# stevengiacalone/triceratops

Hardware: AMD Instinct MI355X
Metric: light-curve-point x sample evals/sec (higher is better)
Workload: dtype f64

## Files before the change

### triceratops_amd/csrc/trx_cells.hpp

```cpp
#pragma once
#include <hip/hip_runtime.h>
#include <math.h>

#include <cstddef>
#include <cstdint>

#include "../../include/trx.h"
#include "trx_device.hpp"
#include "trx_internal.hpp"

namespace {

using namespace trx;

constexpr int MODE_LNL = 0;
constexpr int MODE_GRID = 1;

struct RowsArgs {
    int model, flags;
    const double* time;
    const double* flux;
    int n_time;
    double sigma;
    const double* params;
// ... 373 lines not shown
                }
            }
            hdr[kHdrGrid + lane] = dpt;
            hdr[kHdrG + lane] = g;
        }
        if (lane == 0) {
            hdr[kHdrFlat] = acc;
            hdr[kHdrHmin] = INFINITY;
            hdr[kHdrXmax] = -INFINITY;
            hdr[kHdrProbe] = 1.0;
        }
    }
    {
        const int l = lane, nt = a.n_time;
        bool ok = a.use_stencil && nt >= 64 && a.S >= 2 && a.exptime > 0.0;
        double dt = 0.0, t0 = 0.0;
        if (ok) {
            t0 = a.time[0];
            dt = (a.time[nt - 1] - t0) / (double)(nt - 1);
            double dev = 0.0, big = 0.0;
            for (int j = l; j < nt; j += 64) {
                const double t = a.time[j];
                dev = fmax(dev, fabs(t - fma((double)j, dt, t0)));
                big = fmax(big, fabs(t));
            }
#pragma unroll
            for (int o = 32; o > 0; o >>= 1) {
                dev = fmax(dev, __shfl_xor(dev, o, 64));
                big = fmax(big, __shfl_xor(big, o, 64));
            }
            ok = dt > 0.0 && dev <= 4.0 * 2.220446049250313e-16 * fmax(big, dt);
        }
        const double u = ok ? dt / a.exptime : 1.0;
        ok = ok && u <= 0.3 && 0.5 / u <= 0.5 * kStM + 0.5;
        double w = 0.0, pmax = 0.0;
        if (ok && l <= 2 * kStM + 1) {
            const int i = l - kStM;
            for (int sidx = 1; sidx <= a.S; ++sidx) {
                const double x = (((double)sidx - 0.5) * a.rS - 0.5) / u;
                double num = 1.0, den = 1.0;
                for (int k = -kStM; k <= kStM; ++k) {
                    if (l == 2 * kStM + 1) num *= fabs(x - (double)k);
                    else if (k != i) { num *= x - (double)k; den *= (double)(i - k); }
                }
                if (l == 2 * kStM + 1) pmax = fmax(pmax, num);
                else w += num / den;
            }
            w *= a.rS;
        }
        pmax = __shfl(pmax, 2 * kStM + 1, 64);
        double wabs = (l <= 2 * kStM) ? fabs(w) : 0.0;
#pragma unroll
        for (int o = 32; o > 0; o >>= 1) wabs += __shfl_xor(wabs, o, 64);
        ok = ok && wabs <= 3.0;
        if (l <= 2 * kStM) hdr[kHdrStW + l] = ok ? w : 0.0;
        if (l == 0) {
            double radius = 0.0;
            if (ok) {
                radius = 1.1 * 2.0 * u * ((double)kStM + pow(pmax * 1e15, 1.0 / (2.0 * kStM + 1.0)));
                if (!(radius > 0.0 && radius <= 40.0)) radius = 0.0;
            }
            hdr[kHdrStRadius] = radius;
            if (a.memo) *a.memo = (radius > 0.0) ? 2 : 1;
        }
    }
}

constexpr unsigned long long kUnwrittenBits = 0x7ff8dead0badc0deull;

template <bool SEC>
__device__ __forceinline__ void rowc_body(const RowsArgs& a)
{
    __shared__ RowC rows_out[64];
    const int lane = threadIdx.x;
    const long n = a.n_dev ? *a.n_dev : a.n;
    const long nblk = (n + 63) / 64;
    if (blockIdx.x == gridDim.x - 1) {
        launch_header(a, n);
        return;
    }
    const bool quick = SEC && a.out_sec == nullptr;
    int* list = a.scan_list;
    unsigned long long* count = a.scan_count;
    for (long blk = blockIdx.x; blk < nblk; blk += gridDim.x - 1) {
        const long base = blk * 64;
        const int nb = (int)((n - base < 64) ? (n - base) : 64);
        bool open = false;
        if (lane < nb) {
            RowC c, sc;
            double ysec, fdil;
            row_constants(a, n, base + lane, c, quick, sc, ysec, fdil);
            if (quick) {
#ifndef TRX_SEC_FULL_SCAN
                const Limb L{sc.cle, sc.cld, sc.ced};
                const double ts = __dadd_rn(__dmul_rn(0.1 / 24.0, 12.0), -0.05);
                const double f = exposure_flux(sc, L, ts, 0.0, 1, 1.0, 1.0, false, a.tiers);
                const double m = (f + ysec) / (1.0 + ysec);
                const double depth = 1.0 - (m + fdil) / (1.0 + fdil);
                if (!(depth < 1.5 * a.sigma)) c.excl = 1.0;
                else open = true;
#else
                open = true;
#endif
            }
            const double* src = reinterpret_cast<const double*>(&c);
            double* stage = reinterpret_cast<double*>(&rows_out[lane]);
#pragma unroll
            for (int q = 0; q < kRowDoubles; ++q) stage[q] = src[q];
        }
        if (quick) {
            const unsigned long long mo = __ballot(open);
            if (mo) {
                unsigned long long at = 0;
                if (lane == 0) at = atomicAdd(count, (unsigned long long)__popcll(mo));
                at = __shfl(at, 0, 64);
                const unsigned long long slot = at + (unsigned long long)lanes_below(mo);
                if (open && slot <= (unsigned long long)a.n) list[slot] = (int)(base + lane);
            }
        }
        if (a.mark_unwritten && lane < nb) a.out[base + lane] = __longlong_as_double((long long)kUnwrittenBits);
        __syncthreads();
        {
            const double* src = reinterpret_cast<const double*>(rows_out);
            double* out = a.rowc + base * kRowDoubles;
            for (int i = lane; i < nb * kRowDoubles; i += 64) out[i] = src[i];
        }
        __syncthreads();
    }
}

template <bool SEC>
__global__ __launch_bounds__(64) void rowc_kernel(RowsArgs a)
{
    rowc_body<SEC>(a);
}

__global__ __launch_bounds__(64) void rowc_kernel_star(RowsArgs common, BranchTab bt)
{
    const RowsArgs a = star_args(common, bt, 0);
    if (a.need_sec) rowc_body<true>(a);
    else rowc_body<false>(a);
}

template <int E>
__device__ __forceinline__ void sec_scan_body(const RowsArgs& a)
{
    __shared__ RowC srows[E];
    __shared__ double secmin[E];
    __shared__ int secnan[E];
    const int lane = threadIdx.x;
    const long n = a.n_dev ? *a.n_dev : a.n;
    const bool all_rows = a.out_sec != nullptr;
    const int* list = a.scan_list;
    const long nu = all_rows ? n : (long)*a.scan_count;
    for (long e0 = (long)blockIdx.x * E; e0 < nu; e0 += (long)gridDim.x * E) {
        const int ne = (int)((nu - e0 < E) ? (nu - e0) : E);
        long row = 0;
        double ysec = 0.0, fdil = 0.0;
        if (lane < ne) {
            row = all_rows ? e0 + lane : (long)list[e0 + lane];
            row = (row >= 0 && row < n) ? row : 0;
            RowC unused;
            row_constants<false>(a, n, row, unused, true, srows[lane], ysec, fdil);
            secmin[lane] = INFINITY;
            secnan[lane] = 0;
        }
        __syncthreads();
        for (int it = lane; it < ne * kSecPoints; it += 64) {
            const int ri = it / kSecPoints, j = it - ri * kSecPoints;
            const RowC sc = srows[ri];
            const Limb L{sc.cle, sc.cld, sc.ced};
            double ts = __dadd_rn(__dmul_rn(0.1 / 24.0, (double)j), -0.05);
            if (j == kSecPoints - 1) ts = 0.05;
            const double f = exposure_flux(sc, L, ts, 0.0, 1, 1.0, 1.0, false, a.tiers);
            if (f != f) atomicOr(&secnan[ri], 1);
            else __hip_atomic_fetch_min(&secmin[ri], f, __ATOMIC_RELAXED, __HIP_MEMORY_SCOPE_WORKGROUP);
        }
        __syncthreads();
        if (lane < ne) {
            double m = secnan[lane] ? NAN : secmin[lane];
            m = (m + ysec) / (1.0 + ysec);
            const double secdepth = 1.0 - (m + fdil) / (1.0 + fdil);
            a.rowc[row * kRowDoubles + (kRowDoubles - 1)] = (secdepth < 1.5 * a.sigma) ? 0.0 : 1.0;
            if (a.out_sec) a.out_sec[row] = secdepth;
        }
        __syncthreads();
    }
}

template <int E>
__global__ __launch_bounds__(64) void sec_scan_kernel(RowsArgs a)
{
    sec_scan_body<E>(a);
}

struct BranchMap {
    unsigned char id[TRX_CHAIN_MAX_BRANCHES];
};
__global__ __launch_bounds__(64) void sec_scan_kernel_star(RowsArgs common, BranchTab bt, BranchMap map)
{
    const RowsArgs a = star_args(common, bt, 0, (int)map.id[blockIdx.y]);
    if (!a.need_sec) return;
    sec_scan_body<8>(a);
}
static_assert(offsetof(RowC, excl) == (kRowDoubles - 1) * sizeof(double), "excl is the last field of RowC");

struct CellState {
    double sE[64], cE[64];
    double t[64];
    double facc[64];
    unsigned meta[64];
    unsigned short rel[64];
};
struct StencilState {
    double fc[64 + ((kStM + 7) & ~7)];
    double stw[(2 * kStM + 1 + 7) & ~7];
};
constexpr int kCentreNode = 1023;

__device__ __forceinline__ double fp32_model_slack(double lb, int n_probed, double rs2)
{
    return 1e-5 * sqrt(2.0 * (double)n_probed * rs2 * fmax(lb, 0.0));
}

template <int BITS>
__device__ __forceinline__ int lane_prefix(int cnt, int& total)
{
    int off = 0;
    total = 0;
#pragma unroll
    for (int b = 0; b < BITS; ++b) {
        const unsigned long long m = __ballot((cnt >> b) & 1);
        off += lanes_below(m) << b;
        total += __popcll(m) << b;
    }
    return off;
}

__device__ __forceinline__ double depth_bound(const RowC& c)
{
    const double om4 = 1.0 / (c.cle + c.cld);
    const double u2 = c.ced * om4, u1 = c.cld * om4 - 2.0 * u2;
    double imax = fmax(1.0, 1.0 - u1 - u2);
    if (u2 > 0.0 && u1 < 0.0) imax += u1 * u1 / (4.0 * u2);
    const double d = c.k * c.k * imax * (c.cle + c.cld) * c.rdil * (1.0 + 1e-12);
    return (d >= 0.0) ? d : INFINITY;
}

__device__ __forceinline__ double depth_screen(const double* hdr, double d)
{
    if (!(d < 1.0)) return 0.0;
    int i = (int)ceilf((log10f((float)fmax(d, 1e-30)) + 5.0f) * (63.0f / 5.0f));
    i = i < 0 ? 0 : (i > 63 ? 63 : i);
    if (i > 0 && hdr[kHdrGrid + i - 1] >= d) --i;
    if (hdr[kHdrGrid + i] < d) i = (i < 63) ? i + 1 : 63;
    if (hdr[kHdrGrid + i] < d) return 0.0;
    const double g = 0.5 * hdr[kHdrG + i];
    return g - fma(1e-9, g, 1e-9);
}

__device__ __forceinline__ void tighten_bounds(double* hdr, double h, double x)
{
    if (h < __hip_atomic_load(&hdr[kHdrHmin], __ATOMIC_RELAXED, __HIP_MEMORY_SCOPE_AGENT))
        __hip_atomic_fetch_min(&hdr[kHdrHmin], h, __ATOMIC_RELAXED, __HIP_MEMORY_SCOPE_AGENT);
    if (x > __hip_atomic_load(&hdr[kHdrXmax], __ATOMIC_RELAXED, __HIP_MEMORY_SCOPE_AGENT))
        __hip_atomic_fetch_max(&hdr[kHdrXmax], x, __ATOMIC_RELAXED, __HIP_MEMORY_SCOPE_AGENT);
}

__device__ __forceinline__ void wave_sync()
{
    __builtin_amdgcn_fence(__ATOMIC_RELEASE, "wavefront");
    __builtin_amdgcn_wave_barrier();
    __builtin_amdgcn_fence(__ATOMIC_ACQUIRE, "wavefront");
}

__device__ __forceinline__ int listed_pass_rows(const RowsArgs& a, long rows, int part)
{
    int B = batch_rows(rows, a.n_time, a.forced_B, part == 3 ? a.wave_floor3 : 3200);
    B = B < a.B ? B : a.B;
    if (part == 2 && a.probe_rows > 1) {
        B = a.probe_rows;
        while (B > 1 && rows / B < a.wave_floor) B = (B + 1) / 2;
    }
    return B;
}

#ifndef TRX_ARGS_RELOAD
#define TRX_ARGS_RELOAD 1
#endif
struct StarKernArgs {
    RowsArgs common;
    BranchTab bt;
    int part;
};
template <typename T>
__device__ __forceinline__ const T* kernel_arguments()
{
    typedef const __attribute__((address_space(4))) T* KernArgs;
    KernArgs p = (KernArgs)__builtin_amdgcn_kernarg_segment_ptr();
    asm volatile("" : "+s"(p));
    return (const T*)p;
}

template <int MODE, bool STEP, bool FP32, bool LONG, bool ST, bool PRUNE, int ARGS = 0>
__device__ __forceinline__ void cells_body(const RowsArgs& a_in, const double st_radius)
{
    constexpr int kReload = TRX_ARGS_RELOAD ? ARGS : 0;
    const RowsArgs& a = a_in;
    static_assert(!PRUNE || (MODE == MODE_LNL && !ST), "bounded evaluation: likelihood mode, no stencil");
    extern __shared__ double lds_all[];
    constexpr bool kCarry = TRX_CARRY_CELLS && STEP && !LONG;
    constexpr bool kLazyTiers = TRX_LAZY_TIERS && ST && STEP && LONG && !PRUNE;
    constexpr int W = cells_waves(LONG);
    const int wave = W > 1 ? __builtin_amdgcn_readfirstlane((int)(threadIdx.x >> 6)) : 0;
    double* tier_xw = lds_all;
    double* atab = tier_xw + 2 * kTiers * kTierMaxNodes;
    double* thead = atab + kAtanRanges * kAtanCols;
    double* lds = lds_all + a.wave_off + (size_t)wave * a.wave_doubles;
    const int Bl = LONG ? 1 : a.B;
    RowC* rows = reinterpret_cast<RowC*>(lds);
    double* hacc = lds + (size_t)Bl * kRowDoubles;
    double* hmout = hacc + Bl;
    double* hrem = hmout + Bl;
    double* hlp = hrem + Bl;
    unsigned short* pdesc = reinterpret_cast<unsigned short*>(hlp + Bl);
    constexpr int kCellsWindow = cells_window(LONG);
    unsigned short* winlist = pdesc + kCellsPairs;
    CellState& cs = *reinterpret_cast<CellState*>(winlist + kCellsWindow);
    StencilState& ss = *reinterpret_cast<StencilState*>(&cs + 1);
    const double* tl = LONG ? a.time : (lds_all + a.tl_off);
    const double* fl = LONG ? a.flux : (tl + a.n_time);
    if (a.use_tiers) {
        for (int i = threadIdx.x; i < 2 * kTiers * kTierMaxNodes; i += 64 * W) tier_xw[i] = a.tier_xw[i];
    }
    if (threadIdx.x < kAtanRanges * kAtanCols) atab[threadIdx.x] = kAtanTable[threadIdx.x];
    if (threadIdx.x == 0) {
        thead[0] = a.tiers.radius[0]; thead[1] = a.tiers.radius[1]; thead[2] = a.tiers.radius[2]; thead[3] = a.tiers.radius[3];
        thead[4] = a.tiers.radius[4]; thead[5] = a.tiers.radius[5]; thead[6] = a.tiers.radius[6];
        thead[7] = (double)a.tiers.n[0]; thead[8] = (double)a.tiers.n[1]; thead[9] = (double)a.tiers.n[2];
        thead[10] = (double)a.tiers.n[3]; thead[11] = (double)a.tiers.n[4]; thead[12] = (double)a.tiers.n[5];
        thead[13] = (double)a.tiers.n[6];
    }
    const int lane = W > 1 ? (int)(threadIdx.x & 63) : (int)threadIdx.x;
    constexpr int kWgKeep = (PRUNE && !LONG) ? 8 * kCellsMaxRows : 1;
    __shared__ int wg_keep[kWgKeep];
    __shared__ int wg_nkeep, wg_valid;
    if (PRUNE && !LONG && threadIdx.x == 0) { wg_nkeep = 0; wg_valid = 0x7fffffff; }
    const bool eblike = (a.model == TRX_MODEL_EB) || (a.model == TRX_MODEL_EB_TWIN);
    const double rs2 = a.rs2;
    const int n_time = a.n_time;
    const float inv_nt = __uint_as_float(__builtin_amdgcn_readfirstlane(__float_as_uint(1.0f / (float)n_time)));
    long n = a.n, nbatch = a.nbatch;
    int B = Bl;
    if (a.n_dev) {
        n = *a.n_dev;
        if (!LONG) {
            B = batch_rows(n, n_time, a.forced_B);
            B = B < Bl ? B : Bl;
        }
        nbatch = (n + B - 1) / B;
    }
#ifdef TRX_PHASE_TIMERS
    unsigned long long tm[8] = {0, 0, 0, 0, 0, 0, 0, 0};
    TRX_TICK(t_all);
#endif
    if (!LONG) {
        double* tw = lds_all + a.tl_off;
        for (int j = threadIdx.x; j < n_time; j += 64 * W) {
            tw[j] = a.time[j];
            if (MODE == MODE_LNL) tw[n_time + j] = a.flux[j];
        }
    }
    if (W > 1) __syncthreads();
    const double* hdr = a.rowc + n * kRowDoubles;
    const double flat_sum = (MODE == MODE_LNL && n_time > 0) ? uniform(hdr[kHdrFlat]) : 0.0;
    if (ST && lane <= 2 * kStM) ss.stw[lane] = hdr[kHdrStW + lane];

    long row0 = 0, row1 = n;
    const int* rlist = nullptr;
    if (PRUNE && a.part) {
        const long np = n < kPilotRows ? n : kPilotRows;
        const int* const probe_list = a.probe_list;
        const int* const surv_list = a.surv_list;
        const unsigned long long* const probe_count = a.probe_count;
        const unsigned long long* const surv_count = a.surv_count;
        if (a.part == 1) row1 = np;
        else if (a.part == 2) {
            if (a.split && hdr[kHdrProbe] != 0.0) { rlist = probe_list; row1 = (long)*probe_count; }
            else row0 = np;
        }
        else if (hdr[kHdrProbe] != 0.0) { rlist = surv_list; row1 = (long)*surv_count; }
        else row0 = np;
        if (!LONG && (a.part == 3 || (a.part == 2 && rlist))) B = listed_pass_rows(a, row1 - row0, a.part);
        if (!LONG && a.part == 1 && a.split) B = kPilotB < Bl ? kPilotB : Bl;
        nbatch = (row1 - row0 + B - 1) / B;
    }
    const bool third_two = PRUNE && !LONG && a.part == 3 && a.pstride3 > 1;
    const int pstride = third_two ? a.pstride3 : a.pstride;
    const bool probing = PRUNE && pstride > 1 && hdr[kHdrProbe] != 0.0 &&
                         (a.part == 0 || a.part == 2 || third_two);
    if (PRUNE && a.split && a.part == 2 && !probing) return;
    const BatchPlan bp = LONG ? BatchPlan{} : batch_plan(uniform_long(row1 - row0), __builtin_amdgcn_readfirstlane(B), !PRUNE);
    const long positions = LONG ? (nbatch + 7) / 8 : bp.P;
    const long v0 = (long)(blockIdx.x & 7) + 8 * ((long)(blockIdx.x >> 3) * W + wave);
    unsigned n_skipped = 0, n_pruned = 0;
    for (long v = v0; v < 8 * positions; v += (long)gridDim.x * W) {
        RowsArgs a_again;
        if (kReload == 2) {
            const StarKernArgs* k = kernel_arguments<StarKernArgs>();
            a_again = star_args(k->common, k->bt, k->part);
        }
        const RowsArgs& a = (kReload == 1) ? *kernel_arguments<RowsArgs>() : ((kReload == 2) ? a_again : a_in);
        long base;
        int nb;
        if (LONG) {
            const long batch = (v & 7) * positions + (v >> 3);
            if ((v >> 3) >= positions || batch >= nbatch) continue;
            base = row0 + batch * B;
            nb = (int)((row1 - base < B) ? (row1 - base) : B);
        } else {
            batch_at(bp, v & 7, v >> 3, base, nb);
            base += row0;
            if (base >= row1) continue;
            if (row1 - base < nb) nb = (int)(row1 - base);
        }
        TRX_TICK(t_pro);
        TRX_CENSUS_ADD(kCenBatch, 1);
        int rowid = (int)base + lane;
        if (PRUNE && rlist) {
            if (lane < nb) rowid = rlist[base + lane];
            double* dst = reinterpret_cast<double*>(rows);
            for (int i = lane; i < nb * kRowDoubles; i += 64) {
                const int r = i / kRowDoubles, q = i - r * kRowDoubles;
                dst[i] = a.rowc[(long)rlist[base + r] * kRowDoubles + q];
            }
        } else {
            const double* src = a.rowc + base * kRowDoubles;
            double* dst = reinterpret_cast<double*>(rows);
            for (int i = lane; i < nb * kRowDoubles; i += 64) dst[i] = src[i];
        }
        wave_sync();
        if (lane < nb) {
            const RowC& c = rows[lane];
            hacc[lane] = 0.0;
            hrem[lane] = 0.0;
            double m1 = 1.0;
            m1 = fma(-(1.0 - m1), c.rdil, 1.0);
            hmout[lane] = m1;
        }
        wave_sync();
        unsigned long long skipmask = 0;
        if (MODE == MODE_LNL && a.skip_excl && a.model == TRX_MODEL_EB) {
            skipmask = __ballot(lane < nb && rows[lane].excl != 0.0);
            n_skipped += (unsigned)__popcll(skipmask);
            if (LONG && skipmask) {
                if (lane == 0) a.out[base] = INFINITY;
                wave_sync();
                continue;
            }
        }
        RowC cu;
        if (LONG && !TRX_LONG_ROWS_IN_LDS) {
            const RowC& r0 = rows[0];
            cu.k = uniform(r0.k); cu.t0 = uniform(r0.t0); cu.nmot = uniform(r0.nmot); cu.e = uniform(r0.e);
            cu.Mtr = uniform(r0.Mtr); cu.ax = uniform(r0.ax); cu.ay = uniform(r0.ay); cu.bx = uniform(r0.bx);
            cu.by = uniform(r0.by); cu.cosi = uniform(r0.cosi); cu.cle = uniform(r0.cle); cu.cld = uniform(r0.cld);
            cu.ced = uniform(r0.ced);
            cu.sEt = uniform(r0.sEt); cu.cEt = uniform(r0.cEt);
        }
        double lacc = 0.0;
        bool nonflat = false;
        unsigned long long deadmask = 0;
        bool long_dead = false;
        if (PRUNE && lane < nb) hlp[lane] = a.prune_lp ? a.prune_lp[row_pos(a, rowid)] : 0.0;
#define lp_row (hlp[lane < nb ? lane : 0])
        bool probe_done = false;
        const unsigned long long exclmask = skipmask;
        auto finish_probe = [&]() __attribute__((always_inline)) {
            const bool in_batch = lane < nb;
            const bool is_dead = mask_bit(deadmask, lane), is_excl = mask_bit(exclmask, lane);
            const bool alive = in_batch && !is_dead && !is_excl;
            if (in_batch && !alive) a.out[rowid] = is_excl ? INFINITY : hrem[lane];
            const unsigned long long ma = __ballot(alive);
            if (ma) {
                const int cnt = __popcll(ma);
                int slot = 0;
                if (!LONG) {
                    if (lane == 0) slot = atomicAdd(&wg_nkeep, cnt);
                    slot = __shfl(slot, 0, 64);
                }
                if (!LONG && slot + cnt <= kWgKeep) {
                    if (alive) wg_keep[slot + lanes_below(ma)] = (int)rowid;
                } else {
                    if (!LONG && lane == 0) atomicMin(&wg_valid, slot);
                    unsigned long long at = 0;
                    if (lane == 0) at = atomicAdd(a.surv_count, (unsigned long long)cnt);
                    at = __shfl(at, 0, 64);
                    if (alive) a.surv_list[at + lanes_below(ma)] = (int)rowid;
                }
            }
        };
#ifndef TRX_NO_DEPTH_SCREEN
        if (PRUNE && probing && !a.split) {
            const double hmin_run = __hip_atomic_load(&hdr[kHdrHmin], __ATOMIC_RELAXED, __HIP_MEMORY_SCOPE_AGENT);
            const double xmax_run = __hip_atomic_load(&hdr[kHdrXmax], __ATOMIC_RELAXED, __HIP_MEMORY_SCOPE_AGENT);
            bool shallow = false;
            if (lane < nb && !mask_bit(skipmask, lane)) {
                const double lb = depth_screen(hdr, depth_bound(rows[lane]));
                shallow = hmout[lane] == 1.0 && lb > hmin_run && (a.prune_c0 - lb + lp_row) < xmax_run - 90.0;
#ifdef TRX_PRUNE_NEVER_DEAD
                shallow = false;
#endif
                if (shallow) hrem[lane] = lb;
            }
            const unsigned long long ms = __ballot(shallow);
            if (ms) {
                deadmask |= ms;
                skipmask |= ms;
                n_pruned += (unsigned)__popcll(ms);
                wave_sync();
                if (LONG) {
                    if (lane == 0) a.out[base] = hrem[0];
                    wave_sync();
                    continue;
                }
            }
        }
#endif
        const int nphase = probing ? 2 : 1;
        TRX_TOCK(0, t_pro);

        const unsigned long long rowsmask = (nb >= 64) ? ~0ull : ((1ull << nb) - 1ull);
        const bool all_settled = PRUNE && !LONG && (skipmask & rowsmask) == rowsmask;
        const int ncell = all_settled ? 0 : nb * n_time;
        const int wstep = (PRUNE && !LONG && a.part == 2 && a.probe_rows > 1) ? (ncell > kCellsWindow ? ncell : kCellsWindow) : kCellsWindow;
        for (int win0 = 0; win0 < ncell; win0 += wstep) {
            const int win1 = (win0 + wstep < ncell) ? (win0 + wstep) : ncell;
            for (int phase_no = 0; phase_no < nphase; ++phase_no) {
            TRX_TICK(t_p1);
            int nw = 0;
            for (int c0 = win0; c0 < win1; c0 += 64) {
                const int cell = c0 + lane;
                const bool valid = cell < win1;
                int rr = 0, j = valid ? cell : 0;
                if (!LONG) {
                    rr = valid ? (int)(((float)cell + 0.5f) * inv_nt) : (nb - 1);
                    rr = rr < nb ? rr : nb - 1;
                    j = valid ? (cell - rr * n_time) : 0;
                }
                bool inw = false;
                TRX_CENSUS_ADD(kCenWindowTrip, 1);
                if (PRUNE && !LONG && !__any(valid && !mask_bit(skipmask, rr))) continue;
                if (valid) {
                    const RowC& c = (LONG && !TRX_LONG_ROWS_IN_LDS) ? cu : rows[rr];
                    const double phase = c.nmot * (tl[j] - c.t0);
                    const double dMc = reduce_2pi(phase);
                    const double slack = 1e-15 * fabs(phase);
                    const RowC& cw = rows[rr];
                    inw = in_window(cw.wlo - slack, cw.whi + slack, dMc) && !mask_bit(skipmask, rr);
                    if (MODE == MODE_GRID && (!inw || a.debug_nodes))
                        a.out[(size_t)base * n_time + cell] = a.debug_nodes ? 0.0 : hmout[rr];
                    if (LONG && MODE == MODE_LNL && !inw && phase_no == 0) {
                        const double d = fl[j] - 1.0;
                        lacc = fma(d * d, rs2, lacc);
                    }
                    if (PRUNE) {
                        if (!LONG && inw && phase_no == 0) {
                            const double d = fl[j] - 1.0;
                            __hip_atomic_fetch_add(&hrem[rr], (d * d) * rs2, __ATOMIC_RELAXED, __HIP_MEMORY_SCOPE_WORKGROUP);
                        }
                        if (nphase == 2) {
                            const bool probe = (j % pstride) == (pstride >> 1);
                            inw = inw && (probe == (phase_no == 0));
                        }
                    }
                }
                const unsigned long long mw = __ballot(inw);
                if (inw) winlist[nw + lanes_below(mw)] = (unsigned short)(cell - win0);
                nw += __popcll(mw);
            }
            wave_sync();
            TRX_TOCK(1, t_p1);
            int nheavy = 0;
            for (int sweep = 0; sweep < 2; ++sweep) {
            const int count = sweep ? nheavy : nw;
            const bool halo = ST && sweep == 0 && st_radius > 0.0;
            int carry_j = 0;
            unsigned long long carry_ok = 0;
            int ncarry = 0;
            for (int w0 = 0, step = 64; w0 < count || (kCarry && ncarry > 0); w0 += step) {
                TRX_TICK(t_plan);
                TRX_CENSUS_ADD(sweep ? kCenChunk1 : kCenChunk0, 1);
                bool owned = true;
                const bool carried = kCarry && lane < ncarry;
                if (kCarry) step = 64 - ncarry;
                const int csrc = (lane + 64 - ncarry) & 63;
                const unsigned cmeta = carried ? cs.meta[csrc] : 0u;
                bool valid = carried ? (cmeta & 0x20000u) != 0 : (w0 + lane - ncarry) < count;
                int rel = (int)*(carried ? &cs.rel[csrc] : &winlist[valid ? (w0 + lane - ncarry) : (count - 1)]);
                bool last_chunk = false;
                if (ST && halo) {
                    last_chunk = w0 + 64 >= count;
                    step = last_chunk ? 64 : 64 - kStM;
                    owned = lane < step;
                    if (w0 > 0 && lane < kStM) ss.fc[lane] = ss.fc[kStM + (64 - 2 * kStM) + lane];
                    wave_sync();
                }
                const int cell = win0 + rel;
                int rr = 0, j = cell;
                if (!LONG) {
                    rr = (int)(((float)cell + 0.5f) * inv_nt);
                    rr = rr < nb ? rr : nb - 1;
                    j = cell - rr * n_time;
                }
                const double t = tl[j];
                double fobs = 0.0;
                if (LONG && MODE == MODE_LNL) fobs = fl[j];
                CellPlan pl;
                if (carried) {
                    pl.n = (int)(cmeta >> 18); pl.tier = (int)((cmeta >> 8) & 0xffu) - 1;
                    pl.sE = cs.sE[csrc]; pl.cE = cs.cE[csrc];
                    pl.anchored = (cmeta & 0x10000u) != 0;
                } else if (valid) {
                    const RowC& c = (LONG && !TRX_LONG_ROWS_IN_LDS) ? cu : rows[rr];
#ifndef TRX_PLAN_FULL_SOLVE
                    if (LONG && sweep == 1) pl = plan_all_subexposures<PRUNE>(c, t, a.S);
                    else
#endif
                    pl = plan_cell<false, PRUNE, TRX_TIER_LDS(PRUNE, LONG), kLazyTiers>(c, t, a.exptime, a.S, a.tiers, a.use_tiers != 0,
                                                                                        (ST && sweep == 0) ? st_radius : 0.0, thead);
                    if (STEP && !pl.anchored && pl.n > 0) {
                        kepler_full(c.nmot * (t - c.t0) + c.Mtr, c.e, pl.sE, pl.cE);
                        pl.anchored = true;
                    }
                }
                if (sweep == 0 && a.use_tiers) {
                    const bool heavy = valid && !pl.lazy && pl.tier < 0 && pl.n > 0;
                    const unsigned long long mh = __ballot(heavy && owned);
                    if (heavy && owned) winlist[nheavy + lanes_below(mh)] = (unsigned short)rel;
                    if (heavy) { pl.n = 0; valid = false; }
                    nheavy += __popcll(mh);
                }
                int tier = pl.tier;
                int nodes = (valid && owned) ? pl.n : 0;
                bool st = false, centre = false;
                if (ST && sweep == 0) {
                    const int jleft = __shfl(carry_j, 64 - 2 * kStM + lane, 64), jhere = __shfl(j, lane - kStM, 64);
                    const int jm = (lane < kStM) ? jleft : jhere;
                    const int jp = __shfl(j, lane + kStM, 64);
                    const unsigned long long mok = __ballot(valid);
                    const unsigned long long left = (carry_ok >> (64 - 2 * kStM)) & ((1ull << kStM) - 1ull);
                    const bool inner = (lane >= kStM || (halo && w0 > 0)) && lane + kStM < 64;
                    constexpr unsigned long long kAll = (1ull << (2 * kStM + 1)) - 1ull;
                    const unsigned long long field = (lane >= kStM) ? (mok >> (lane - kStM)) : (((mok << kStM) | left) >> lane);
                    st = inner && owned && valid && pl.n > 0 && pl.st_ok && jm == j - kStM && jp == j + kStM &&
                         (field & kAll) == kAll;
                    const unsigned long long mst = __ballot(st);
                    unsigned long long dil = mst;
#pragma unroll
                    for (int i = 1; i <= kStM; ++i) dil |= (mst << i) | (mst >> i);
                    centre = valid && ((dil >> lane) & 1ull);
                    const unsigned long long mnext = __ballot(valid && pl.n > 0 && pl.st_ok) >> (64 - kStM);
                    const int kk = lane - (64 - 2 * kStM);
                    if (halo && !last_chunk && valid && !centre && kk >= 0 && kk < kStM && (mnext & ((2ull << kk) - 1ull)) != 0) {
                        if (pl.n > 0) centre = true;
                        else ss.fc[kStM + lane] = 1.0;
                    }
                    if (st) nodes = 0;
                    carry_j = j;
                    carry_ok = mok;
                    if (kLazyTiers) {
                        const bool need = pl.lazy && nodes > 0;
                        if (__any(need)) {
                            if (need) {
                                const RowC& c = (LONG && !TRX_LONG_ROWS_IN_LDS) ? cu : rows[rr];
                                plan_tiers(c, a.exptime, pl, thead);
                                tier = pl.tier;
                                nodes = pl.n;
                            }
                        }
                    }
                }
                const bool direct = kLazyTiers && ST && sweep == 0 && !__any(nodes > 0);
                if (direct) {
                    if (centre) {
                        const RowC& c = (LONG && !TRX_LONG_ROWS_IN_LDS) ? cu : rows[rr];
                        const double ce = pl.cE - c.e;
                        const double X = fma(c.ax, ce, c.bx * pl.sE);
                        const double Y = fma(c.ay, ce, c.by * pl.sE);
                        const double yc = Y * c.cosi;
                        const double z2 = fma(X, X, yc * yc);
                        const double opp = 1.0 + c.k;
                        double f = 1.0;
                        if (Y >= 0.0 && z2 < opp * opp) {
                            const Limb L{c.cle, c.cld, c.ced};
                            f = disc_flux<FP32, TRX_ATAN_TAB(PRUNE, LONG)>(sqrt_fast(z2), c.k, L, atab);
                        } else if (z2 != z2) {
                            f = z2;
                        }
                        ss.fc[kStM + lane] = f;
                    }
                    wave_sync();
                }
                if (kCarry) wave_sync();
                if (!direct) {
                    cs.sE[lane] = pl.sE; cs.cE[lane] = pl.cE;
                    cs.t[lane] = t;
                    cs.facc[lane] = 0.0;
                    cs.meta[lane] = (unsigned)rr | ((unsigned)(tier + 1) << 8) | (pl.anchored ? 0x10000u : 0u) |
                                    (valid ? 0x20000u : 0u) | ((unsigned)pl.n << 18);
                    if (kCarry) cs.rel[lane] = (unsigned short)rel;
                }
                TRX_TOCK(2, t_plan);
                TRX_TICK(t_a);
                int ldone = 64;
                const int ncells = __popcll(__ballot(nodes > 0 || (ST && centre)));
                int per = ncells > 0 ? kCellsPairs / ncells - (ST ? 1 : 0) : kCellsPairs;
                per = per > 1000 ? 1000 : (per < 1 ? 1 : per);
                for (int s0 = 0; !direct && __any(s0 < nodes || (ST && s0 == 0 && centre)); s0 += per) {
                    int cnt = nodes - s0;
                    cnt = cnt < 0 ? 0 : (cnt > per ? per : cnt);
                    TRX_CENSUS_ADD(kCenPass, 1);
                    const int extra = (ST && s0 == 0 && centre) ? 1 : 0;
                    int total;
                    const int off = (sweep == 0 && a.use_tiers) ? lane_prefix<4>(cnt + extra, total)
                                                                : lane_prefix<10>(cnt + extra, total);
                    for (int si = 0; si < cnt; ++si) pdesc[off + si] = (unsigned short)(lane | (si << 6));
                    if (extra) pdesc[off + cnt] = (unsigned short)(lane | (kCentreNode << 6));
                    wave_sync();
                    if (kCarry && !(ST && halo) && s0 == 0 && w0 + step < count && total >= 64 && !__any(nodes > per)) {
                        const int whole = total & ~63;
                        const int l0 = __popcll(__ballot(off + cnt + extra <= whole));
                        if (l0 >= 1 && l0 < 64 && (64 - (total - whole)) > (64 - l0)) {
                            ldone = l0;
                            total = __builtin_amdgcn_readlane(off, l0);
                        }
                    }
                    for (int p0 = 0; p0 < total; p0 += 64) {
                        const int p = p0 + lane;
                        TRX_CENSUS_ADD(kCenPairTrip, 1);
                        TRX_CENSUS_ADD(kCenPairLanes, (unsigned long long)(total - p0 < 64 ? total - p0 : 64));
                        if (p < total) {
                            const int d = (int)pdesc[p];
                            const int h = d & 63;
                            const bool at_centre = ST && (d >> 6) == kCentreNode;
                            const int s = at_centre ? 0 : s0 + (d >> 6);
                            const unsigned meta = cs.meta[h];
                            const RowC& c = (LONG && !TRX_LONG_ROWS_IN_LDS) ? cu : rows[meta & 0xffu];
                            const int ht = (int)((meta >> 8) & 0xffu) - 1;
                            double sE = cs.sE[h], cE = cs.cE[h];
                            if (!at_centre) {
                                const double frac = (ht < 0) ? fma((double)(s + 1) - 0.5, a.rS, -0.5)
                                                             : tier_xw[2 * (ht * kTierMaxNodes + s)];
                                const double dM = c.nmot * (a.exptime * frac);
                                bool have = false;
                                if (STEP && (meta & 0x10000u)) have = kepler_step<PRUNE>(dM, c.e, sE, cE);
                                if (!have) {
                                    TRX_CENSUS_ADD(kCenKeplerFullPair, 1);
                                    kepler_full(c.nmot * ((cs.t[h] + a.exptime * frac) - c.t0) + c.Mtr, c.e, sE, cE);
                                }
                            }
                            const double ce = cE - c.e;
                            const double X = fma(c.ax, ce, c.bx * sE);
                            const double Y = fma(c.ay, ce, c.by * sE);
                            const double yc = Y * c.cosi;
                            const double z2 = fma(X, X, yc * yc);
                            const double opp = 1.0 + c.k;
                            double f = 1.0;
                            if (Y >= 0.0 && z2 < opp * opp) {
                                const Limb L{c.cle, c.cld, c.ced};
                                f = disc_flux<FP32, TRX_ATAN_TAB(PRUNE, LONG)>(sqrt_fast(z2), c.k, L, atab);
                            } else if (z2 != z2) {
                                f = z2;
                            }
                            if (at_centre) {
                                ss.fc[kStM + h] = f;
                            } else {
                                const double term = (ht < 0) ? f : tier_xw[2 * (ht * kTierMaxNodes + s) + 1] * (1.0 - f);
                                if (ht < 0 || term != 0.0)
                                    __hip_atomic_fetch_add(&cs.facc[h], term, __ATOMIC_RELAXED, __HIP_MEMORY_SCOPE_WORKGROUP);
                            }
                        }
                    }
                    wave_sync();
                }
                TRX_TOCK(3, t_a);
                TRX_TICK(t_rest);
                if (MODE == MODE_GRID && a.debug_nodes) {
                    const int spent = nodes + ((ST && centre) ? 1 : 0);
                    if (spent > 0 && lane < ldone) atomicAdd(&a.out[(size_t)base * n_time + cell], (double)spent);
                } else if (valid && owned && lane < ldone) {
                    const RowC& c = (LONG && !TRX_LONG_ROWS_IN_LDS) ? cu : rows[rr];
                    double fsum = cs.facc[lane];
                    if (ST && st) {
                        fsum = 0.0;
#pragma unroll
                        for (int i = -kStM; i <= kStM; ++i) fsum = fma(ss.stw[i + kStM], 1.0 - ss.fc[kStM + lane + i], fsum);
                    }
                    const double deficit = (pl.n == 0) ? 0.0 : ((ST && st) ? fsum : ((tier < 0) ? 1.0 - fsum / a.dS : fsum));
                    const RowC& cd = rows[rr];
                    const double m = fma(-deficit, cd.rdil, 1.0);
                    if (MODE == MODE_GRID) {
                        a.out[(size_t)base * n_time + cell] = m;
                    } else {
                        if (LONG) {
                            const double d = fobs - m;
                            lacc = fma(d * d, rs2, lacc);
                            nonflat = nonflat || (m != 1.0);
                        } else {
                            const double f = fl[j];
                            const double contrib = ((1.0 - m) * ((f - m) + (f - 1.0))) * rs2;
                            if (contrib != 0.0)
                                __hip_atomic_fetch_add(&hacc[rr], contrib, __ATOMIC_RELAXED, __HIP_MEMORY_SCOPE_WORKGROUP);
                            if (PRUNE && nphase == 2 && phase_no == 0) {
                                const double d1 = f - 1.0;
                                __hip_atomic_fetch_add(&hrem[rr], -(d1 * d1) * rs2, __ATOMIC_RELAXED, __HIP_MEMORY_SCOPE_WORKGROUP);
                            }
                        }
                    }
                }
                if (kCarry) ncarry = 64 - ldone;
                TRX_TOCK(5, t_rest);
            }
            }
            wave_sync();
            if (PRUNE && nphase == 2 && phase_no == 0) {
                const double* hdr_b = a.rowc + n * kRowDoubles;
                const double hmin_run = __hip_atomic_load(&hdr_b[kHdrHmin], __ATOMIC_RELAXED, __HIP_MEMORY_SCOPE_AGENT);
                const double xmax_run = __hip_atomic_load(&hdr_b[kHdrXmax], __ATOMIC_RELAXED, __HIP_MEMORY_SCOPE_AGENT);
                if (LONG) {
                    double lb = 0.5 * wave_sum(lacc);
                    lb -= fma(1e-9, fabs(lb), 1e-9);
                    if (FP32) lb -= fp32_model_slack(lb, n_time / pstride + 1, rs2);
                    const double lp0 = hlp[0];
                    long_dead = hmout[0] == 1.0 && lb > hmin_run && (a.prune_c0 - lb + lp0) < xmax_run - 90.0;
                    if (long_dead) {
                        if (lane == 0) a.out[base] = lb;
                        ++n_pruned;
                        break;
                    }
                } else {
                    bool dead = false;
                    if (lane < nb && !mask_bit(skipmask, lane)) {
// ... 252 lines not shown
```

Before: 46.20 billion.

## Compute in-transit index ranges analytically for long stencil cells instead of scanning

```diff
diff --git a/triceratops_amd/csrc/trx_cells.hpp b/triceratops_amd/csrc/trx_cells.hpp
--- a/triceratops_amd/csrc/trx_cells.hpp
+++ b/triceratops_amd/csrc/trx_cells.hpp
@@ -699,6 +699,44 @@
     return (const T*)p;
 }
 
+constexpr int kMaxWindowRanges = 16;
+__device__ __noinline__ int window_ranges(double wlo, double whi, double t0, double nmot, const double* time, int n_time,
+                                          int win0, int win1, int* rng)
+{
+    const int lane = (int)(threadIdx.x & 63);
+    if (wlo > whi) return 0;
+    const double tf = time[0], tl = time[n_time - 1];
+    const double dt = (tl - tf) / (double)(n_time - 1);
+    if (!(wlo >= -3.0 && whi <= 3.0 && whi - wlo <= kPi && nmot > 0.0 && nmot < INFINITY && fabs(t0) < INFINITY &&
+          kTwoPi / nmot >= 4.0 * dt))
+        return -1;
+    const double mag = fabs(tf) + fabs(tl) + 2.0 * fabs(t0) + (fabs(wlo) + fabs(whi)) / nmot;
+    if (!(1e-13 * mag <= 0.25 * dt)) return -1;
+    const double rev = 1.0 / kTwoPi;
+    const double nlo = floor((nmot * (tf - t0) - whi) * rev), nhi = ceil((nmot * (tl - t0) - wlo) * rev);
+    if (!(nhi - nlo < (double)kMaxWindowRanges)) return -1;
+    const int nr = (int)(nhi - nlo) + 1;
+    if (lane < nr) {
+        const double orb = kTwoPi * (nlo + (double)lane);
+        const double xlo = ((t0 + (wlo + orb) / nmot) - tf) / dt, xhi = ((t0 + (whi + orb) / nmot) - tf) / dt;
+        const int lo = (int)fmin(fmax(ceil(xlo) - 1.0, 0.0), (double)n_time);
+        const int hi = (int)fmax(fmin(floor(xhi) + 1.0, (double)(n_time - 1)), -1.0);
+        auto inw = [&](int j) {
+            if (j < lo || j > hi) return false;
+            const double phase = nmot * (time[j] - t0);
+            const double slack = 1e-15 * fabs(phase);
+            return in_window(wlo - slack, whi + slack, reduce_2pi(phase));
+        };
+        int l2 = inw(lo) ? lo : (inw(lo + 1) ? lo + 1 : lo + 2);
+        int h2 = inw(hi) ? hi : (inw(hi - 1) ? hi - 1 : hi - 2);
+        l2 = l2 > win0 ? l2 : win0;
+        h2 = h2 < win1 - 1 ? h2 : win1 - 1;
+        rng[2 * lane] = l2;
+        rng[2 * lane + 1] = h2;
+    }
+    return nr;
+}
+
 template <int MODE, bool STEP, bool FP32, bool LONG, bool ST, bool PRUNE, int ARGS = 0>
 __device__ __forceinline__ void cells_body(const RowsArgs& a_in, const double st_radius)
 {
@@ -708,6 +746,7 @@
     extern __shared__ double lds_all[];
     constexpr bool kCarry = TRX_CARRY_CELLS && STEP && !LONG;
     constexpr bool kLazyTiers = TRX_LAZY_TIERS && ST && STEP && LONG && !PRUNE;
+    constexpr bool kRanges = ST && STEP && LONG && !PRUNE;
     constexpr int W = cells_waves(LONG);
     const int wave = W > 1 ? __builtin_amdgcn_readfirstlane((int)(threadIdx.x >> 6)) : 0;
     double* tier_xw = lds_all;
@@ -936,6 +975,42 @@
             for (int phase_no = 0; phase_no < nphase; ++phase_no) {
             TRX_TICK(t_p1);
             int nw = 0;
+            int nranges = -1;
+            int* rng = reinterpret_cast<int*>(pdesc);
+            auto rng_at = [&](int i) __attribute__((always_inline)) { return rng[i]; };
+            if (kRanges && st_radius > 0.0) {
+                const RowC& c = (LONG && !TRX_LONG_ROWS_IN_LDS) ? cu : rows[0];
+                nranges = __builtin_amdgcn_readfirstlane(window_ranges(rows[0].wlo, rows[0].whi, c.t0, c.nmot, tl, n_time,
+                                                                       win0, win1, rng));
+                wave_sync();
+            }
+            if (kRanges && nranges >= 0) {
+                int prev = win0;
+                for (int r = 0; r <= nranges; ++r) {
+                    int lo = (r < nranges) ? rng_at(2 * r) : win1;
+                    const int hi = (r < nranges) ? rng_at(2 * r + 1) : win1 - 1;
+                    lo = lo > prev ? lo : prev;
+                    if (r < nranges && hi < lo) continue;
+                    for (int c0 = win0 + ((prev - win0) & ~63); c0 < lo; c0 += 64) {
+                        const int j = c0 + lane;
+                        if (j >= prev && j < lo) {
+                            if (MODE == MODE_GRID) a.out[(size_t)base * n_time + j] = a.debug_nodes ? 0.0 : hmout[0];
+                            if (MODE == MODE_LNL) {
+                                const double d = fl[j] - 1.0;
+                                lacc = fma(d * d, rs2, lacc);
+                            }
+                        }
+                    }
+                    for (int k = lo + lane; k <= hi; k += 64) {
+                        winlist[nw + (k - lo)] = (unsigned short)(k - win0);
+                        if (MODE == MODE_GRID && a.debug_nodes) a.out[(size_t)base * n_time + k] = 0.0;
+                    }
+                    if (hi >= lo) {
+                        nw += hi - lo + 1;
+                        prev = hi + 1;
+                    }
+                }
+            } else
             for (int c0 = win0; c0 < win1; c0 += 64) {
                 const int cell = c0 + lane;
                 const bool valid = cell < win1;
```

New measurement: 47.42 billion, median of 6. 1.03x the previous value.
